# THUDM/CogView

Hardware: AMD Instinct MI355X
Metric: train tokens/sec/node (seq1089, 4B GPT) at 1/2/4/8 MI355X; % MFMA roofline (higher is better)
Workload: dtype fp16

## Files before the change

cogview_amd/_lib.py:

```python
import ctypes as C
import os

_HERE = os.path.dirname(os.path.abspath(__file__))
LIB_PATH = os.environ.get("COGVIEW_HIP_LIB") or os.path.join(_HERE, "lib", "libcogview_hip.so")

F16, BF16, F32 = 0, 1, 2
EPI_BIAS, EPI_GELU, EPI_DGELU, EPI_DROPOUT, EPI_ABSMAX, EPI_ACCUM, EPI_COLSUM = 1, 2, 4, 8, 16, 32, 64
EPI_GELU_DAUX, EPI_MULAUX = 128, 256

_ERR = {1: "bad argument (shape / alignment / dtype)", 2: "kernel launch failure", 3: "unsupported combination"}


class CogviewHipError(RuntimeError):
    pass


class GemmDesc(C.Structure):
    _fields_ = [
        ("dtype", C.c_int), ("trans_a", C.c_int), ("trans_b", C.c_int),
        ("M", C.c_int), ("N", C.c_int), ("K", C.c_int),
        ("A", C.c_void_p), ("lda", C.c_int),
        ("B", C.c_void_p), ("ldb", C.c_int),
        ("C", C.c_void_p), ("ldc", C.c_int),
        ("out_f32", C.c_int), ("flags", C.c_int),
# ... 89 lines not shown


CONV_4X4_S2, CONV_1X1, CONVT_4X4_S2, CONV_3X3_S1 = 0, 1, 2, 3

_vp, _i, _f, _u64, _i64, _sz = C.c_void_p, C.c_int, C.c_float, C.c_uint64, C.c_int64, C.c_size_t

SIGNATURES = {
    "cogv_version": (_i, []),
    "cogv_arch": (C.c_char_p, []),
    "cogv_gemm": (_i, [C.POINTER(GemmDesc), _vp]),
    "cogv_gemm_workspace_bytes": (_sz, [C.POINTER(GemmDesc)]),
    "cogv_gemm_pick_splitk": (_i, [_i, _i, _i]),
    "cogv_gemm_grouped": (_i, [C.POINTER(GemmDesc), _i, _vp]),
    "cogv_gemm_colsum_rows": (_i, [_i]),
    "cogv_colsum_finalize": (_i, [_i, _vp, _i, _i, _vp, _i, _vp]),
    "cogv_gemm_pick_splitk_tiles": (_i, [_i, _i]),
    "cogv_sandwich_ln_fwd": (_i, [_i, _vp, _vp, _vp, _vp, _vp, _vp, _vp, _vp, _vp, _i, _i, _f, _i, _vp]),
    "cogv_sandwich_ln_bwd": (_i, [_i, _vp, _vp, _vp, _vp, _vp, _vp, _vp, _vp, _vp, _vp, _i, _i, _i, _f, _u64, _u64,
                                  _vp, _sz, _i, _vp]),
    "cogv_sandwich_ln_bwd_marked": (_i, [_i, _vp, _vp, _vp, _vp, _vp, _vp, _vp, _vp, _vp, _vp, _i, _i, _i, _f, _vp, _sz, _i, _vp]),
    "cogv_ln_bwd_workspace_bytes": (_sz, [_i, _i]),
    "cogv_sandwich_ln_bwd_pair": (_i, [_i, _vp, _vp, _vp, _vp, _vp, _vp, _vp, _vp, _vp, _vp, _vp, _vp, _vp, _vp, _vp, _vp, _vp, _i, _i, _i, _f,
                                       _vp, _sz, _vp]),
    "cogv_ln_bwd_pair_workspace_bytes": (_sz, [_i, _i]),
    "cogv_ln_bwd_num_blocks": (_i, [_i]),
    "cogv_ln_bwd_plan": (_i, [_i, _i, _i, _f, _i, _i, C.POINTER(C.c_int)]),
    "cogv_ln_bwd_pair_plan": (_i, [_i, _i, _f, C.POINTER(C.c_int)]),
    "cogv_gemm_reserve_cus": (_i, [_i]),
    "cogv_attention_fwd": (_i, [C.POINTER(AttnDesc), _vp]),
    "cogv_attention_bwd": (_i, [C.POINTER(AttnDesc), _vp]),
    "cogv_gemv_ln": (_i, [C.POINTER(GemmDesc), C.POINTER(LnPrologue), _vp]),
    "cogv_gemv_attn": (_i, [C.POINTER(GemmDesc), _vp, _i, _i, _vp]),
    "cogv_attention_decode": (_i, [C.POINTER(AttnDecodeDesc), _vp]),
    "cogv_attention_decode_workspace_bytes": (_sz, [_i, _i, _i]),
    "cogv_attention_keep_bits_bytes": (_sz, [_i, _i, _i, _i]),
    "cogv_sparse_slot_reduce": (_i, [_i, _vp, _vp, _vp, _vp, _vp, _i64, _i, _i64, _i, _i, _i, _i, _i, _i, _i, _vp]),
    "cogv_embedding_fwd": (_i, [_i, _vp, _vp, _i64, _i64, _vp, _vp, _vp, _i64, _vp, _vp, _i64, _i, _f, _u64, _u64, _i, _vp]),
    "cogv_embedding_bwd": (_i, [_i, _vp, _vp, _vp, _i64, _i64, _vp, _vp, _i64, _vp, _i64, _i, _f, _u64, _u64, _vp, _sz, _i, _vp]),
    "cogv_embedding_bwd_workspace_bytes": (_sz, [_i64, _i64]),
    "cogv_gelu_fwd": (_i, [_i, _vp, _vp, _sz, _vp]),
    "cogv_gelu_bwd": (_i, [_i, _vp, _vp, _vp, _sz, _vp]),
    "cogv_dropout": (_i, [_i, _vp, _vp, _sz, _f, _u64, _u64, _vp, _vp]),
    "cogv_add": (_i, [_i, _vp, _vp, _vp, _sz, _vp, _vp]),
    "cogv_add_stream": (_i, [_i, _vp, _vp, _vp, _sz, _vp, _vp]),
    "cogv_scale": (_i, [_i, _vp, _vp, _sz, _f, _vp]),
    "cogv_absmax": (_i, [_i, _vp, _sz, _vp, _vp]),
# ... 41 lines not shown
```

cogview_amd/csrc/layernorm.hip:

```cpp
#include "common.cuh"
#include "cogview_hip.h"

#include <algorithm>
#include <cstdlib>

namespace {

struct LnFwdArgs {
  const void* x; const void* gamma; const void* beta; const void* res;
  void* y; float* mean; float* rstd;
  const float* absmax_in; float* absmax_out;
  int rows, h; float eps;
};

template <typename T, int NV, int MODE>
__global__ __launch_bounds__(256) void ln_fwd_kernel(const LnFwdArgs p) {
  typedef Row8<T, MODE == 1> XR;
  typedef Row8<T, MODE == 2> YR;
  const int lane = threadIdx.x & 63;
  const int wave_global = blockIdx.x * 4 + (threadIdx.x >> 6);
  const int nwaves = gridDim.x * 4;
  float eps = p.eps;
  if (p.absmax_in) { const float c = *p.absmax_in * 0.125f; eps = p.eps * c * c; }
  const float inv_h = 1.0f / (float)p.h;
// ... 332 lines not shown
#endif
      if (act && row < p.rows) {
        float o[8];
#pragma unroll
        for (int i = 0; i < 8; ++i) o[i] = rstd3[r] * fmaf(-xh3[r][i], n2, gy3[r][i] - n1);
        if (p.marked) {
#pragma unroll
          for (int i = 0; i < 8; ++i) o[i] = marked_dropped(aor[r], i) ? 0.f : o[i] * p.keep_scale;
        }
        (void)TR::st(p.d_ao, (size_t)row * p.h + col, o, 0u);
#pragma unroll
        for (int i = 0; i < 8; ++i) cs[i] += o[i];
      }
    }
  }
  if (act) {
    float* o2 = p.partial2 + (size_t)blockIdx.x * 3 * p.h + col;
    float* o3 = p.partial3 + (size_t)blockIdx.x * 3 * p.h + col;
#pragma unroll
    for (int i = 0; i < 8; ++i) { o2[i] = dg2[i]; o2[p.h + i] = db2[i]; o3[i] = dg3[i]; o3[p.h + i] = db3[i]; o3[2 * p.h + i] = cs[i]; }
  }
}

template <typename T>
__global__ __launch_bounds__(1024) void ln_bwd_reduce_kernel(const float* partial, int nblk, int h, void* dgamma,
                                                            void* dbeta, void* colsum, int accumulate) {
  const int c = blockIdx.x * 64 + (threadIdx.x & 63);
  const int part = threadIdx.x >> 6;
  const int set = blockIdx.y;
  T* out = reinterpret_cast<T*>(set == 0 ? dgamma : set == 1 ? dbeta : colsum);
  __shared__ float red[16][64];
  float s = 0.f;
  if (c < h && out) {
    float t[8] = {0.f, 0.f, 0.f, 0.f, 0.f, 0.f, 0.f, 0.f};
    int b = part;
    for (; b + 7 * 16 < nblk; b += 8 * 16) {
#pragma unroll
      for (int u = 0; u < 8; ++u) t[u] += partial[((size_t)(b + 16 * u) * 3 + set) * h + c];
    }
    for (; b < nblk; b += 16) t[0] += partial[((size_t)b * 3 + set) * h + c];
    s = ((t[0] + t[1]) + (t[2] + t[3])) + ((t[4] + t[5]) + (t[6] + t[7]));
  }
  red[part][threadIdx.x & 63] = s;
  __syncthreads();
  if (part == 0 && c < h && out) {
    float t = 0.f;
#pragma unroll
    for (int i = 0; i < 16; ++i) t += red[i][threadIdx.x];
    if (accumulate) t += HT<T>::to_f(out[c]);
    out[c] = HT<T>::from_f(t);
  }
}

template <typename T, int NV, int MODE> void launch_fwd_m(const LnFwdArgs& a, int blocks, hipStream_t st) {
  static const int resident = [] {
    int per_cu = 0, dev = 0;
    hipDeviceProp_t prop;
    if (hipOccupancyMaxActiveBlocksPerMultiprocessor(&per_cu, ln_fwd_kernel<T, NV, MODE>, 256, 0) != hipSuccess || per_cu < 1) return 4096;
    if (hipGetDevice(&dev) != hipSuccess || hipGetDeviceProperties(&prop, dev) != hipSuccess) return 4096;
    return per_cu * prop.multiProcessorCount;
  }();
  if (blocks > resident) blocks = resident;
  hipLaunchKernelGGL((ln_fwd_kernel<T, NV, MODE>), dim3(blocks), dim3(256), 0, st, a);
}
template <typename T, int NV> void launch_fwd(const LnFwdArgs& a, int mode, int blocks, hipStream_t st) {
  if (mode == COGV_LN_STREAM_IN) launch_fwd_m<T, NV, 1>(a, blocks, st);
  else if (mode == COGV_LN_STREAM_OUT) launch_fwd_m<T, NV, 2>(a, blocks, st);
  else launch_fwd_m<T, NV, 0>(a, blocks, st);
}

#define NV_SWITCH(FN, T, nv, ...)                          \
  switch (nv) {                                            \
// ... 33 lines not shown
  if (marked && drop && mode != COGV_LN_STREAM_IN) {
    p.marked = true;
    if (wide && sw.marked_rows != 4) { p.rows_in_flight = 2; p.lean = lean_ok; }
  } else if (lean_ok) { p.rows_in_flight = 2; p.lean = true; }
  else if (wide && (drop || (mode == COGV_LN_STREAM_IN && sw.stream_in_rows == 2))) p.rows_in_flight = 2;
  const int cap = wide ? (p.rows_in_flight == 2 && drop ? 512 : 256) : 2560 / nw;
  p.blocks = p.lean ? ln_bwd_grid(rows, 2, 768) : ln_bwd_grid(rows, 4, cap);
  return p;
}
LnBwdPlan ln_bwd_pair_plan(int rows, int h, bool drop) {
  return LnBwdPlan{2, false, drop, ln_bwd_grid(rows, 2, ln_switches().pair_blocks), 64 * ((h + 511) / 512)};
}

inline bool ln_bwd_args_ok(int mode, int rows, int h, float dropout_p) {
  return mode >= 0 && mode <= 2 && rows > 0 && h > 0 && !(h & 7) && h <= 4096 && dropout_p >= 0.f && dropout_p < 1.f;
}
int ln_plan_out(const LnBwdPlan& p, int out[5]) {
  out[0] = p.rows_in_flight, out[1] = p.lean, out[2] = p.marked, out[3] = p.blocks, out[4] = p.threads;
  return COGV_OK;
}
template <typename T> void ln_bwd_reduce(const float* partial, int nblk, int h, void* dgamma, void* dbeta, void* colsum,
                                         int accumulate, hipStream_t st) {
  if (!dgamma && !dbeta && !colsum) return;
  hipLaunchKernelGGL((ln_bwd_reduce_kernel<T>), dim3((h + 63) / 64, 3), dim3(1024), 0, st, partial, nblk, h, dgamma, dbeta, colsum, accumulate);
}
constexpr int ln_form(int mode, int r, bool lean, bool mark) { return mode * 100 + r * 10 + lean * 2 + mark; }
template <typename T> int ln_bwd_run(const LnBwdArgs& a, int mode, const LnBwdPlan& p, void* dgamma, void* dbeta, void* colsum,
                                     int accumulate, hipStream_t st) {
  switch (ln_form(mode, p.rows_in_flight, p.lean, p.marked)) {
#define LN_FORM(MODE, R, LEAN, MARK) \
  case ln_form(MODE, R, LEAN, MARK): hipLaunchKernelGGL((ln_bwd_kernel<T, R, MODE, LEAN, MARK>), dim3(p.blocks), dim3(p.threads), 0, st, a); break;
    LN_FORM(0, 4, false, false) LN_FORM(0, 2, false, false) LN_FORM(0, 4, false, true) LN_FORM(0, 2, false, true)
    LN_FORM(1, 4, false, false) LN_FORM(1, 2, false, false)
    LN_FORM(2, 4, false, false) LN_FORM(2, 2, false, false) LN_FORM(2, 4, false, true) LN_FORM(2, 2, false, true)
    LN_FORM(2, 2, true, false) LN_FORM(2, 2, true, true)
#undef LN_FORM
    default: return COGV_ERR_UNSUPPORTED;
  }
  ln_bwd_reduce<T>(a.partial, p.blocks, a.h, dgamma, dbeta, colsum, accumulate, st);
  return cogv_check_launch();
}
template <typename T> int ln_bwd_pair_run(const LnPairArgs& a, const LnBwdPlan& p, void* dgamma2, void* dbeta2, void* dgamma3,
                                          void* dbeta3, void* colsum, int accumulate, hipStream_t st) {
  hipLaunchKernelGGL((ln_bwd_pair_kernel<T, 2>), dim3(p.blocks), dim3(p.threads), 0, st, a);
  ln_bwd_reduce<T>(a.partial2, p.blocks, a.h, dgamma2, dbeta2, nullptr, accumulate, st);
  ln_bwd_reduce<T>(a.partial3, p.blocks, a.h, dgamma3, dbeta3, colsum, accumulate, st);
  return cogv_check_launch();
}

}

extern "C" int cogv_ln_bwd_num_blocks(int rows) {
  const int b = (rows + 3) / 4;
  return b < 1 ? 1 : (b > 1024 ? 1024 : b);
}
extern "C" size_t cogv_ln_bwd_workspace_bytes(int rows, int h) {
  return (size_t)cogv_ln_bwd_num_blocks(rows) * 3 * (size_t)h * sizeof(float);
}
extern "C" int cogv_ln_bwd_plan(int stream_mode, int rows, int h, float dropout_p, int marked, int has_add_in, int out[5]) {
  if (marked && stream_mode == COGV_LN_STREAM_IN) return COGV_ERR_ARG;
  if (!ln_bwd_args_ok(stream_mode, rows, h, dropout_p)) return COGV_ERR_ARG;
  return ln_plan_out(ln_bwd_plan(stream_mode, rows, h, ln_thr16(dropout_p) != 0, marked != 0, has_add_in != 0), out);
}
extern "C" int cogv_ln_bwd_pair_plan(int rows, int h, float dropout_p, int out[5]) {
  if (!ln_bwd_args_ok(COGV_LN_ALL_T, rows, h, dropout_p)) return COGV_ERR_ARG;
  if ((h + 511) / 512 < 4) return COGV_ERR_UNSUPPORTED;
  return ln_plan_out(ln_bwd_pair_plan(rows, h, ln_thr16(dropout_p) != 0), out);
}

// ... 33 lines not shown
  return dtype == COGV_F16 ? ln_bwd_run<f16_t>(a, stream_mode, plan, dgamma, dbeta, colsum, accumulate_param_grads, st)
                           : ln_bwd_run<bf16_t>(a, stream_mode, plan, dgamma, dbeta, colsum, accumulate_param_grads, st);
}

extern "C" int cogv_sandwich_ln_bwd(int dtype, const void* dy, const void* x, const void* gamma, const float* mean,
                                    const float* rstd, const void* add_in, void* dx, void* dgamma, void* dbeta,
                                    void* colsum, int accumulate_param_grads, int rows, int h, float dropout_p,
                                    uint64_t seed, uint64_t stream_id, void* workspace, size_t workspace_bytes,
                                    int stream_mode, void* stream) {
  return ln_bwd_impl(dtype, dy, x, gamma, mean, rstd, add_in, dx, dgamma, dbeta, colsum, accumulate_param_grads, rows, h,
                     dropout_p, seed, stream_id, workspace, workspace_bytes, stream_mode, stream, 0);
}

extern "C" int cogv_sandwich_ln_bwd_marked(int dtype, const void* dy, const void* x, const void* gamma, const float* mean,
                                           const float* rstd, const void* add_in, void* dx, void* dgamma, void* dbeta,
                                           void* colsum, int accumulate_param_grads, int rows, int h, float dropout_p,
                                           void* workspace, size_t workspace_bytes, int stream_mode, void* stream) {
  if (stream_mode == COGV_LN_STREAM_IN) return COGV_ERR_ARG;
  return ln_bwd_impl(dtype, dy, x, gamma, mean, rstd, add_in, dx, dgamma, dbeta, colsum, accumulate_param_grads, rows, h,
                     dropout_p, 0, 0, workspace, workspace_bytes, stream_mode, stream, dropout_p > 0.f ? 1 : 0);
}

extern "C" size_t cogv_ln_bwd_pair_workspace_bytes(int rows, int h) { return 2 * cogv_ln_bwd_workspace_bytes(rows, h); }
extern "C" int cogv_sandwich_ln_bwd_pair(int dtype, const void* dc, const void* y, const void* gamma2, const float* mean2,
                                         const float* rstd2, const void* dout, void* dy, void* dgamma2, void* dbeta2,
                                         const void* ao, const void* gamma3, const float* mean3, const float* rstd3, void* d_ao,
                                         void* dgamma3, void* dbeta3, void* colsum, int accumulate_param_grads, int rows, int h,
                                         float dropout_p, void* workspace, size_t workspace_bytes, void* stream) {
  if (dtype != COGV_F16 && dtype != COGV_BF16) return COGV_ERR_UNSUPPORTED;
  if (!ln_bwd_args_ok(COGV_LN_ALL_T, rows, h, dropout_p)) return COGV_ERR_ARG;
  if (!dc || !y || !gamma2 || !mean2 || !rstd2 || !dout || !dy || !ao || !gamma3 || !mean3 || !rstd3 || !d_ao || !workspace) return COGV_ERR_ARG;
  if (workspace_bytes < cogv_ln_bwd_pair_workspace_bytes(rows, h)) return COGV_ERR_ARG;
  if (((uintptr_t)dc | (uintptr_t)y | (uintptr_t)gamma2 | (uintptr_t)dout | (uintptr_t)dy | (uintptr_t)ao | (uintptr_t)gamma3 | (uintptr_t)d_ao) & 15)
    return COGV_ERR_ARG;
  if ((h + 511) / 512 < 4) return COGV_ERR_UNSUPPORTED;
  const uint32_t thr16 = ln_thr16(dropout_p);
  float* const partial = reinterpret_cast<float*>(workspace);
  const LnPairArgs a{dc, y, gamma2, mean2, rstd2, dout, dy, ao, gamma3, mean3, rstd3, d_ao, partial,
                     partial + (size_t)cogv_ln_bwd_num_blocks(rows) * 3 * (size_t)h, rows, h, thr16 != 0, 65536.0f / (65536.0f - (float)thr16)};
  const LnBwdPlan plan = ln_bwd_pair_plan(rows, h, thr16 != 0);
  hipStream_t st = reinterpret_cast<hipStream_t>(stream);
  return dtype == COGV_F16 ? ln_bwd_pair_run<f16_t>(a, plan, dgamma2, dbeta2, dgamma3, dbeta3, colsum, accumulate_param_grads, st)
                           : ln_bwd_pair_run<bf16_t>(a, plan, dgamma2, dbeta2, dgamma3, dbeta3, colsum, accumulate_param_grads, st);
}
```

cogview_amd/functional.py:

```python
import contextlib
import math
import os

import torch

from . import ops
from .mpu import mappings
from .mpu import random as mpu_random
from .mpu.initialize import get_model_parallel_group, mp_rank_or_0, mp_world_size_or_1


def grad_buffer(p):
    if p.grad is None:
        p.grad = torch.zeros_like(p)
    return p.grad


def grad_accumulate(*params):
    params = [p for p in params if p is not None]
    arenas = [getattr(p, "_cogv_arena", (None,))[0] for p in params]
    if params and all(a is not None and a is arenas[0] for a in arenas):
        return not arenas[0].take_fresh(params)
    for p, a in zip(params, arenas):
        if a is not None:
            a.ensure_zeroed(p)
# ... 487 lines not shown
                                    slot_ao, residual=x, absmax_out=slot_y, save_stats=keep is not None)
    c, m2, r2 = ops.sandwich_ln_fwd(y, layer.post_attention_layernorm.weight, layer.post_attention_layernorm.bias,
                                    eps, slot_y, save_stats=keep is not None)
    f4 = mlp_m.dense_h_to_4h.weight.shape[0]
    u = torch.empty((rows, f4), dtype=a.dtype, device=dev) if keep is not None else None
    g = ops.gemm(c.view(rows, h), mlp_m.dense_h_to_4h.weight, bias=mlp_m.dense_h_to_4h.bias, gelu=True, gelu_daux=u)
    slot_mo = ops.new_absmax_slot(dev)
    if mp == 1:
        mo = ops.gemm(g, mlp_m.dense_4h_to_h.weight, bias=mlp_m.dense_4h_to_h.bias, dropout=d_mo, absmax=slot_mo)
    else:
        mo = _row_parallel_chunked(g, mlp_m.dense_4h_to_h.weight, mlp_m.dense_4h_to_h.bias if rank == 0 else None, d_mo, slot_mo)
    slot_out = ops.new_absmax_slot(dev)
    out, m4, r4 = ops.sandwich_ln_fwd(mo.view(b, s, h), layer.fourth_layernorm.weight, layer.fourth_layernorm.bias,
                                      eps, slot_mo, residual=y, absmax_out=slot_out, save_stats=keep is not None)
    if keep is not None:
        keep.x, keep.a, keep.qkv, keep.att, keep.lse, keep.ao, keep.y, keep.c = x, a, qkv, att, lse, ao, y, c
        keep.u, keep.g, keep.mo = u, g, mo
        keep.st1, keep.st2, keep.st3, keep.st4 = (m1, r1), (m2, r2), (m3, r3), (m4, r4)
        keep.d_attn, keep.d_ao, keep.d_mo, keep.kbits = d_attn, d_ao, d_mo, kbits
    return out, slot_out


LN_BWD_PAIR = os.environ.get("COGV_LN_BWD_PAIR", "1") != "0"


def _layer_backward(layer, kp, dout, sep):
    att_m, mlp_m = layer.attention, layer.mlp
    b, s, h = kp.x.shape
    rows = b * s
    npp = att_m.num_attention_heads_per_partition
    hp = npp * 64
    G = grad_buffer
    ln1, ln2, ln3, ln4 = (layer.input_layernorm, layer.post_attention_layernorm, layer.third_layernorm,
                          layer.fourth_layernorm)
    W1, b1, W2, b2 = mlp_m.dense_h_to_4h.weight, mlp_m.dense_h_to_4h.bias, mlp_m.dense_4h_to_h.weight, mlp_m.dense_4h_to_h.bias
    Wq, bq, Wo, bo = att_m.query_key_value.weight, att_m.query_key_value.bias, att_m.dense.weight, att_m.dense.bias
    dout = dout if dout.is_contiguous() else dout.contiguous()

    marked = mp_world_size_or_1() == 1 and os.environ.get("COGV_LN_BWD_MARKED", "1") != "0"
    d_mo = ops.sandwich_ln_bwd(dout, kp.mo, ln4.weight, *kp.st4, dropout=kp.d_mo, dgamma=G(ln4.weight), marked=marked,
                               dbeta=G(ln4.bias), colsum=G(b2), accumulate=grad_accumulate(ln4.weight, ln4.bias, b2)).view(rows, h)
    mp = mp_world_size_or_1()
    wgrads = []

    def _wg(dy_, x_, w_):
        if mp == 1:
            defer_weight_grad(dy_, x_, w_, owner=layer)
        else:
            wgrads.append((dy_, x_, w_))
    du = ops.gemm(d_mo, W2, trans_b=True, mul_aux=kp.u, colsum_out=G(b1),
                  colsum_accumulate=grad_accumulate(b1))
    _wg(d_mo, kp.g, W2)
    dc = ops.gemm(du, W1, trans_b=True)
    _wg(du, kp.c.view(rows, h), W1)
    if mp > 1:
        work = _mp_allreduce_start(dc)
        with _room_for_collective():
            _launch_weight_grads(wgrads)
        del wgrads[:]
        _mp_allreduce_finish(work)
    p_ao = 0.0 if kp.d_ao is None else float(kp.d_ao[0])
    if LN_BWD_PAIR and ops.ln_bwd_pair_supported(h) and (marked or p_ao == 0.0):
        dy, d_ao = ops.sandwich_ln_bwd_pair(dc.view(b, s, h), kp.y, ln2.weight, *kp.st2, dout, kp.ao, ln3.weight, *kp.st3,
                                            dropout_p=p_ao, dgamma2=G(ln2.weight), dbeta2=G(ln2.bias), dgamma3=G(ln3.weight),
# ... 4 lines not shown
        dy = ops.sandwich_ln_bwd(dc.view(b, s, h), kp.y, ln2.weight, *kp.st2, add_in=dout, dgamma=G(ln2.weight),
                                 dbeta=G(ln2.bias), accumulate=grad_accumulate(ln2.weight, ln2.bias))
        d_ao = ops.sandwich_ln_bwd(dy, kp.ao, ln3.weight, *kp.st3, dropout=kp.d_ao, dgamma=G(ln3.weight), marked=marked,
                                   dbeta=G(ln3.bias), colsum=G(bo), accumulate=grad_accumulate(ln3.weight, ln3.bias, bo)).view(rows, h)
    d_att = ops.gemm(d_ao, Wo, trans_b=True).view(b, s, npp, 64)
    _wg(d_ao, kp.att.view(rows, hp), Wo)
    qkv = kp.qkv
    q = qkv[:, :, 0:hp].view(b, s, npp, 64)
    k = qkv[:, :, hp:2 * hp].view(b, s, npp, 64)
    v = qkv[:, :, 2 * hp:].view(b, s, npp, 64)
    dqkv = torch.empty_like(qkv)
    ops.attention_bwd(d_att, q, k, v, kp.att, kp.lse, sep=sep, dropout=kp.d_attn,
                      dq=dqkv[:, :, 0:hp].view(b, s, npp, 64), dk=dqkv[:, :, hp:2 * hp].view(b, s, npp, 64),
                      dv=dqkv[:, :, 2 * hp:].view(b, s, npp, 64), colsum_out=G(bq), colsum_accumulate=grad_accumulate(bq),
                      keep_bits=getattr(kp, "kbits", None))
    dqkv2 = dqkv.view(rows, 3 * hp)
    da = ops.gemm(dqkv2, Wq, trans_b=True)
    _wg(dqkv2, kp.a.view(rows, h), Wq)
    if mp > 1:
        work = _mp_allreduce_start(da)
        with _room_for_collective():
            _launch_weight_grads(wgrads)
        _mp_allreduce_finish(work)
    dx = ops.sandwich_ln_bwd(da.view(b, s, h), kp.x, ln1.weight, *kp.st1, add_in=dy, dgamma=G(ln1.weight),
                             dbeta=G(ln1.bias), accumulate=grad_accumulate(ln1.weight, ln1.bias))
    return dx


class _WgradEntry:
    __slots__ = ("dy", "x", "w", "owner", "t0", "trows", "tiles_n", "acc")

    def __init__(self, dy, x, w, owner):
        self.dy, self.x, self.w, self.owner = dy, x, w, owner
        self.t0, self.acc = 0, None
        self.trows, self.tiles_n = (w.shape[0] + 255) // 256, (w.shape[1] + 255) // 256

    def tiles_left(self):
        return (self.trows - self.t0) * self.tiles_n


def plan_wgrad_chunks(entries, budget):
    out, left = [], budget
    for i, (t0, trows, tiles_n, out_rows) in enumerate(entries):
        if t0 >= trows:
            continue
        n = trows - t0
# ... 106 lines not shown
def nested_backward():
    _NESTED_OUTER.append(torch._C._current_graph_task_id())
    try:
        yield
    finally:
        _NESTED_OUTER.pop()


def defer_weight_grad(dy, x, w, owner=None):
    q = _WGRADS
    task = torch._C._current_graph_task_id()
    root = _NESTED_OUTER[0] if _NESTED_OUTER else task
    if root >= 0 and q.root != root:
        q.entries, q.callbacks, q.new_tiles = [], [], 0
        q.root, q.hooked = root, set()
    if task >= 0 and task not in q.hooked:
        torch.autograd.Variable._execution_engine.queue_callback(_flush_at_end_of_backward)
        q.hooked.add(task)
    q.add(dy, x, w, owner)


class _TransformerLayer(torch.autograd.Function):
    @staticmethod
    def forward(ctx, x, absmax_x, layer, sep, drops, recompute, on_backward_done):
        xc = x if x.is_contiguous() else x.contiguous()
        keep = None if recompute else _LayerCtx()
        out, slot = _layer_forward(layer, xc, absmax_x, sep, drops, keep)
        ctx.layer, ctx.sep, ctx.drops, ctx.recompute, ctx.keep = layer, sep, drops, recompute, keep
        ctx.done_cb = on_backward_done
        if recompute:
            piece, ctx.x_shape = mpu_random.partition_activation(xc)
            ctx.save_for_backward(piece, absmax_x)
        ctx.mark_non_differentiable(slot)
        return out, slot

    @staticmethod
    def backward(ctx, dout, _):
        keep = ctx.keep
        if ctx.recompute:
            xc, absmax_x = ctx.saved_tensors
            xc = mpu_random.gather_activation(xc, ctx.x_shape)
            keep = _LayerCtx()
            _layer_forward(ctx.layer, xc, absmax_x, ctx.sep, ctx.drops, keep)
        dx = _layer_backward(ctx.layer, keep, dout, ctx.sep)
        ctx.keep = None
        if ctx.done_cb is not None:
            _WGRADS.callbacks.append((ctx.done_cb, ctx.layer))
        idx = getattr(ctx.layer, "_cogv_index", 0)
        if idx % wgrad_group_layers(ctx.layer) == 0:
            flush_weight_grads(final=(idx == 0))
        return dx, None, None, None, None, None, None


_DECODE_FUSE_ENV = _os.environ.get("COGV_DECODE_FUSE_COMBINE")


_DECODE_CHAIN_MAX_ROWS = min(8, max(0, int(_os.environ.get("COGV_DECODE_CHAIN_MAX_ROWS", "4"))))


def _decode_fuse_combine():
    if _DECODE_FUSE_ENV is not None:
        return _DECODE_FUSE_ENV != "0"
    return not torch.cuda.is_current_stream_capturing()


def decode_chain_supported(tr, batch):
    h = tr.layers[0].input_layernorm.weight.shape[0]
    return (mp_world_size_or_1() == 1 and batch <= _DECODE_CHAIN_MAX_ROWS and h % 512 == 0 and h <= 4096
            and tr.layers[0].input_layernorm.weight.dtype in (torch.float16, torch.bfloat16))


def decode_chain(tr, h0, absmax0, slots, emb_weight):
    b, s, h = h0.shape
    assert s == 1
# ... 22 lines not shown
        z, z_absmax, post, res = mo, None, (layer.fourth_layernorm.weight, layer.fourth_layernorm.bias), y
    fl = tr.final_layernorm
    logits, _ = ops.gemv_ln(z, emb_weight, None, fl.weight, fl.bias, fl.eps, z_absmax, post, res)
    return logits.view(b, 1, emb_weight.shape[0])


def transformer_layer_kv(layer, x, absmax_x, sep, kv_slot):
    xc = x if x.is_contiguous() else x.contiguous()
    if absmax_x is None:
        absmax_x = ops.absmax(xc)
    out, slot = _layer_forward(layer, xc, absmax_x, sep, (None, None, None), None, kv_slot=kv_slot)
    out._cogv_absmax = slot
    return out


def transformer_layer(layer, x, absmax_x, sep, training, recompute=False, on_backward_done=None):
    p_attn = layer.attention.attention_dropout.p
    p_out = layer.attention.output_dropout.p
    p_mlp = layer.mlp.dropout.p
    drops = (_drop(p_attn, training, attention=True), _drop(p_out, training), _drop(p_mlp, training))
    if absmax_x is None:
        absmax_x = ops.absmax(x if x.is_contiguous() else x.contiguous())
    if torch.is_grad_enabled() and x.requires_grad:
        out, slot = _TransformerLayer.apply(x, absmax_x, layer, sep, drops, recompute, on_backward_done)
    else:
        out, slot = _layer_forward(layer, x if x.is_contiguous() else x.contiguous(), absmax_x, sep, drops, None)
    out._cogv_absmax = slot
    return out
```

cogview_amd/ops.py:

```python
import ctypes as C
import os

import torch

from . import _lib as L

_DT = {torch.float16: L.F16, torch.bfloat16: L.BF16, torch.float32: L.F32}


def dt_code(t):
    try:
        return _DT[t.dtype if isinstance(t, torch.Tensor) else t]
    except KeyError:
        raise L.CogviewHipError(f"unsupported dtype {t.dtype if isinstance(t, torch.Tensor) else t}")


def _need_gpu(*ts):
    for t in ts:
        if t is not None and not t.is_cuda:
            raise L.CogviewHipError(
                "cogview_amd ops run only on an MI355X (HIP) device: got a CPU tensor and there is no CPU fallback")


def _p(t):
# ... 420 lines not shown

def sandwich_ln_bwd_pair(dc, y, gamma2, mean2, rstd2, dout, ao, gamma3, mean3, rstd3, dropout_p=0.0, dgamma2=None, dbeta2=None,
                         dgamma3=None, dbeta3=None, colsum=None, accumulate=False):
    _need_gpu(dc, y, ao)
    h = y.shape[-1]
    dc2, y2, do2, ao2 = dc.reshape(-1, h), y.reshape(-1, h), dout.reshape(-1, h), ao.reshape(-1, h)
    assert dc2.is_contiguous() and y2.is_contiguous() and do2.is_contiguous() and ao2.is_contiguous()
    if y.dtype != torch.float32 or dout.dtype != torch.float32 or dc.dtype != gamma2.dtype or ao.dtype != gamma2.dtype:
        raise L.CogviewHipError("Sandwich-LN backward pair: y / dout must be the fp32 stream, dc / ao the 16-bit storage type")
    rows = y2.shape[0]
    dy = torch.empty_like(y2)
    d_ao = torch.empty_like(ao2)
    lib = L.lib()
    ws = workspace("ln_bwd_pair", lib.cogv_ln_bwd_pair_workspace_bytes(rows, h), y.device)
    nb = rows * h * (2 + 4 + 4 + 4 + 2 + 2)
    with timed_launch("layernorm", 0.0, nb, lambda: "ln_bwd pair: stream in + add, then stream out" + (" + dropout from marked zeros" if dropout_p > 0.0 else "")):
        L.check(lib.cogv_sandwich_ln_bwd_pair(dt_code(gamma2), _p(dc2), _p(y2), _p(gamma2), _p(mean2), _p(rstd2), _p(do2), _p(dy),
                                              _p(dgamma2), _p(dbeta2), _p(ao2), _p(gamma3), _p(mean3), _p(rstd3), _p(d_ao),
                                              _p(dgamma3), _p(dbeta3), _p(colsum), int(accumulate), rows, h, float(dropout_p),
                                              _p(ws), ws.numel(), _stream()), "cogv_sandwich_ln_bwd_pair")
    return dy.view(y.shape), d_ao.view(ao.shape)


def attention_executed_flops(b, H, s_q, s_k, sep=0, dense=True):
    nq, nk = (s_q + 63) // 64, (s_k + 63) // 64
    if dense:
        off = s_k - s_q
        sep_i = int(sep) if isinstance(sep, int) else 0
        blocks = 0
        for i in range(nq):
            last_key = max(min(s_q, 64 * i + 64) - 1 + off, sep_i - 1)
            blocks += max(0, min(nk, last_key // 64 + 1))
    else:
        blocks = nq * nk
    return float(b) * H * blocks * 4.0 * 64 * 64 * 64


def _attn_strides(t):
    assert t.dim() == 4 and t.shape[-1] == 64 and t.stride(3) == 1 and (t.stride(2) == 64 or t.shape[2] == 1)
    return t.stride(0), t.stride(1)


def _attn_desc(q, k, v, o, sep, dropout):
    d = L.AttnDesc()
    d.dtype = dt_code(q)
    d.B, d.s_q, d.H = q.shape[0], q.shape[1], q.shape[2]
# ... 436 lines not shown
```

include/cogview_hip.h:

```cpp
#ifndef COGVIEW_HIP_H
#define COGVIEW_HIP_H

#include <stddef.h>
#include <stdint.h>

#ifdef __cplusplus
extern "C" {
#endif

#define COGV_F16 0
#define COGV_BF16 1
#define COGV_F32 2

int cogv_version(void);
const char* cogv_arch(void);

#define COGV_EPI_BIAS 1
#define COGV_EPI_GELU 2
#define COGV_EPI_DGELU 4
#define COGV_EPI_DROPOUT 8
#define COGV_EPI_ABSMAX 16
#define COGV_EPI_ACCUM 32
#define COGV_EPI_COLSUM 64

// ... 38 lines not shown
} cogv_ln_prologue;
int cogv_gemv_ln(const cogv_gemm_desc* d, const cogv_ln_prologue* ln, void* stream);
int cogv_gemv_attn(const cogv_gemm_desc* d, const void* partials, int heads, int capacity, void* stream);

#define COGV_LN_ALL_T 0
#define COGV_LN_STREAM_IN 1
#define COGV_LN_STREAM_OUT 2
int cogv_sandwich_ln_fwd(int dtype, const void* x, const void* gamma, const void* beta, const void* residual,
                         void* y, float* mean, float* rstd, const float* absmax_in, float* absmax_out,
                         int rows, int h, float eps, int stream_mode, void* stream);
int cogv_sandwich_ln_bwd(int dtype, const void* dy, const void* x, const void* gamma, const float* mean,
                         const float* rstd, const void* add_in, void* dx, void* dgamma, void* dbeta, void* colsum,
                         int accumulate_param_grads, int rows, int h, float dropout_p, uint64_t seed,
                         uint64_t stream_id, void* workspace, size_t workspace_bytes, int stream_mode, void* stream);
int cogv_sandwich_ln_bwd_marked(int dtype, const void* dy, const void* x, const void* gamma, const float* mean,
                                const float* rstd, const void* add_in, void* dx, void* dgamma, void* dbeta, void* colsum,
                                int accumulate_param_grads, int rows, int h, float dropout_p, void* workspace,
                                size_t workspace_bytes, int stream_mode, void* stream);
int cogv_sandwich_ln_bwd_pair(int dtype, const void* dc, const void* y, const void* gamma2, const float* mean2,
                              const float* rstd2, const void* dout, void* dy, void* dgamma2, void* dbeta2,
                              const void* ao, const void* gamma3, const float* mean3, const float* rstd3, void* d_ao,
                              void* dgamma3, void* dbeta3, void* colsum, int accumulate_param_grads, int rows, int h,
                              float dropout_p, void* workspace, size_t workspace_bytes, void* stream);
size_t cogv_ln_bwd_pair_workspace_bytes(int rows, int h);
size_t cogv_ln_bwd_workspace_bytes(int rows, int h);
int cogv_ln_bwd_num_blocks(int rows);
int cogv_ln_bwd_plan(int stream_mode, int rows, int h, float dropout_p, int marked, int has_add_in, int out[5]);
int cogv_ln_bwd_pair_plan(int rows, int h, float dropout_p, int out[5]);

typedef struct cogv_attn_desc {
  int dtype; int B, H, s_q, s_k, head_dim; int sep;
  float scale;
  float dropout_p; uint64_t seed; uint64_t stream_id;
  const void* q; const void* k; const void* v; void* o;
  const void* dout; void* dq; void* dk; void* dv;
  float* lse; float* dvec;
  long long q_bs, k_bs, v_bs, o_bs, do_bs, dq_bs, dk_bs, dv_bs;
  int q_rs, k_rs, v_rs, o_rs, do_rs, dq_rs, dk_rs, dv_rs;
  float* colsum_partial;
  const int* kv_index; long long kv_index_bs;
  long long kv_index_gs; int sparse_window, sparse_pivots; float sparse_pivot_bias;
  void* keep_bits;
  const void* mask; long long mask_bs;
} cogv_attn_desc;
int cogv_attention_fwd(const cogv_attn_desc* d, void* stream);
int cogv_attention_bwd(const cogv_attn_desc* d, void* stream);
// ... 104 lines not shown
```

Measured before the change: 43980.

## Pair LN1 backward with the layer below's LN4 backward across layer boundaries

Fuses the current layer's LN1 backward with the next-lower layer's LN4 backward into one pair kernel. It hands the resulting d_mo and the un-reduced partial sums down to that layer, which then runs only the parameter-grad reduction instead of a full LN4 backward pass. The non-open pair path also merges its two reduce launches into a single 6-set reduce kernel. The aim is to cut a memory-bound LN pass and launches per layer, at the cost of cross-layer state, an extra partial buffer allocation per layer, and a fallback path when the gradient identity check fails.

```diff
diff --git a/cogview_amd/_lib.py b/cogview_amd/_lib.py
--- a/cogview_amd/_lib.py
+++ b/cogview_amd/_lib.py
@@ -135,6 +135,9 @@
     "cogv_ln_bwd_workspace_bytes": (_sz, [_i, _i]),
     "cogv_sandwich_ln_bwd_pair": (_i, [_i, _vp, _vp, _vp, _vp, _vp, _vp, _vp, _vp, _vp, _vp, _vp, _vp, _vp, _vp, _vp, _vp, _vp, _i, _i, _i, _f,
                                        _vp, _sz, _vp]),
+    "cogv_sandwich_ln_bwd_pair_open": (_i, [_i, _vp, _vp, _vp, _vp, _vp, _vp, _vp, _vp, _vp, _i, _vp, _vp, _vp, _vp, _vp, _vp, _sz, _i, _i, _f,
+                                            _vp, _sz, _vp]),
+    "cogv_ln_bwd_reduce": (_i, [_i, _vp, _i, _i, _vp, _vp, _vp, _i, _vp]),
     "cogv_ln_bwd_pair_workspace_bytes": (_sz, [_i, _i]),
     "cogv_ln_bwd_num_blocks": (_i, [_i]),
     "cogv_ln_bwd_plan": (_i, [_i, _i, _i, _f, _i, _i, C.POINTER(C.c_int)]),
diff --git a/cogview_amd/csrc/layernorm.hip b/cogview_amd/csrc/layernorm.hip
--- a/cogview_amd/csrc/layernorm.hip
+++ b/cogview_amd/csrc/layernorm.hip
@@ -378,16 +378,23 @@
   }
 }
 
+struct LnReduceArgs {
+  const float* partial[2];
+  void* out[6];
+  int nblk, h, accumulate[2];
+};
 template <typename T>
-__global__ __launch_bounds__(1024) void ln_bwd_reduce_kernel(const float* partial, int nblk, int h, void* dgamma,
-                                                            void* dbeta, void* colsum, int accumulate) {
+__global__ __launch_bounds__(1024) void ln_bwd_reduce_kernel(const LnReduceArgs a) {
   const int c = blockIdx.x * 64 + (threadIdx.x & 63);
   const int part = threadIdx.x >> 6;
-  const int set = blockIdx.y;
-  T* out = reinterpret_cast<T*>(set == 0 ? dgamma : set == 1 ? dbeta : colsum);
+  const int which = blockIdx.y / 3, set = blockIdx.y % 3;
+  const float* partial = a.partial[which];
+  const int nblk = a.nblk, h = a.h;
+  T* out = reinterpret_cast<T*>(a.out[blockIdx.y]);
+  if (!out) return;
   __shared__ float red[16][64];
   float s = 0.f;
-  if (c < h && out) {
+  if (c < h) {
     float t[8] = {0.f, 0.f, 0.f, 0.f, 0.f, 0.f, 0.f, 0.f};
     int b = part;
     for (; b + 7 * 16 < nblk; b += 8 * 16) {
@@ -399,11 +406,11 @@
   }
   red[part][threadIdx.x & 63] = s;
   __syncthreads();
-  if (part == 0 && c < h && out) {
+  if (part == 0 && c < h) {
     float t = 0.f;
 #pragma unroll
     for (int i = 0; i < 16; ++i) t += red[i][threadIdx.x];
-    if (accumulate) t += HT<T>::to_f(out[c]);
+    if (a.accumulate[which]) t += HT<T>::to_f(out[c]);
     out[c] = HT<T>::from_f(t);
   }
 }
@@ -483,7 +490,8 @@
 template <typename T> void ln_bwd_reduce(const float* partial, int nblk, int h, void* dgamma, void* dbeta, void* colsum,
                                          int accumulate, hipStream_t st) {
   if (!dgamma && !dbeta && !colsum) return;
-  hipLaunchKernelGGL((ln_bwd_reduce_kernel<T>), dim3((h + 63) / 64, 3), dim3(1024), 0, st, partial, nblk, h, dgamma, dbeta, colsum, accumulate);
+  const LnReduceArgs a{{partial, nullptr}, {dgamma, dbeta, colsum, nullptr, nullptr, nullptr}, nblk, h, {accumulate, 0}};
+  hipLaunchKernelGGL((ln_bwd_reduce_kernel<T>), dim3((h + 63) / 64, 3), dim3(1024), 0, st, a);
 }
 constexpr int ln_form(int mode, int r, bool lean, bool mark) { return mode * 100 + r * 10 + lean * 2 + mark; }
 template <typename T> int ln_bwd_run(const LnBwdArgs& a, int mode, const LnBwdPlan& p, void* dgamma, void* dbeta, void* colsum,
@@ -502,10 +510,13 @@
   return cogv_check_launch();
 }
 template <typename T> int ln_bwd_pair_run(const LnPairArgs& a, const LnBwdPlan& p, void* dgamma2, void* dbeta2, void* dgamma3,
-                                          void* dbeta3, void* colsum, int accumulate, hipStream_t st) {
+                                          void* dbeta3, void* colsum, int accumulate, bool open, hipStream_t st) {
   hipLaunchKernelGGL((ln_bwd_pair_kernel<T, 2>), dim3(p.blocks), dim3(p.threads), 0, st, a);
-  ln_bwd_reduce<T>(a.partial2, p.blocks, a.h, dgamma2, dbeta2, nullptr, accumulate, st);
-  ln_bwd_reduce<T>(a.partial3, p.blocks, a.h, dgamma3, dbeta3, colsum, accumulate, st);
+  if (open) ln_bwd_reduce<T>(a.partial2, p.blocks, a.h, dgamma2, dbeta2, nullptr, accumulate, st);
+  else if (dgamma2 || dbeta2 || dgamma3 || dbeta3 || colsum) {
+    const LnReduceArgs r{{a.partial2, a.partial3}, {dgamma2, dbeta2, nullptr, dgamma3, dbeta3, colsum}, p.blocks, a.h, {accumulate, accumulate}};
+    hipLaunchKernelGGL((ln_bwd_reduce_kernel<T>), dim3((a.h + 63) / 64, 6), dim3(1024), 0, st, r);
+  }
   return cogv_check_launch();
 }
 
@@ -585,24 +596,53 @@
 }
 
 extern "C" size_t cogv_ln_bwd_pair_workspace_bytes(int rows, int h) { return 2 * cogv_ln_bwd_workspace_bytes(rows, h); }
+static int ln_bwd_pair_impl(int dtype, const void* dc, const void* y, const void* gamma2, const float* mean2,
+                            const float* rstd2, const void* dout, void* dy, void* dgamma2, void* dbeta2,
+                            const void* ao, const void* gamma3, const float* mean3, const float* rstd3, void* d_ao,
+                            void* dgamma3, void* dbeta3, void* colsum, int accumulate_param_grads, int rows, int h,
+                            float dropout_p, float* partial3, void* workspace, size_t workspace_bytes, void* stream) {
+  if (dtype != COGV_F16 && dtype != COGV_BF16) return COGV_ERR_UNSUPPORTED;
+  if (!ln_bwd_args_ok(COGV_LN_ALL_T, rows, h, dropout_p)) return COGV_ERR_ARG;
+  if (!dc || !y || !gamma2 || !mean2 || !rstd2 || !dout || !dy || !ao || !gamma3 || !mean3 || !rstd3 || !d_ao || !workspace) return COGV_ERR_ARG;
+  if (workspace_bytes < (partial3 ? cogv_ln_bwd_workspace_bytes(rows, h) : cogv_ln_bwd_pair_workspace_bytes(rows, h))) return COGV_ERR_ARG;
+  if (((uintptr_t)dc | (uintptr_t)y | (uintptr_t)gamma2 | (uintptr_t)dout | (uintptr_t)dy | (uintptr_t)ao | (uintptr_t)gamma3 | (uintptr_t)d_ao |
+       (uintptr_t)partial3) & 15)
+    return COGV_ERR_ARG;
+  if ((h + 511) / 512 < 4) return COGV_ERR_UNSUPPORTED;
+  const uint32_t thr16 = ln_thr16(dropout_p);
+  float* const partial = reinterpret_cast<float*>(workspace);
+  const bool open = partial3 != nullptr;
+  const LnPairArgs a{dc, y, gamma2, mean2, rstd2, dout, dy, ao, gamma3, mean3, rstd3, d_ao, partial,
+                     open ? partial3 : partial + (size_t)cogv_ln_bwd_num_blocks(rows) * 3 * (size_t)h, rows, h, thr16 != 0,
+                     65536.0f / (65536.0f - (float)thr16)};
+  const LnBwdPlan plan = ln_bwd_pair_plan(rows, h, thr16 != 0);
+  hipStream_t st = reinterpret_cast<hipStream_t>(stream);
+  return dtype == COGV_F16 ? ln_bwd_pair_run<f16_t>(a, plan, dgamma2, dbeta2, dgamma3, dbeta3, colsum, accumulate_param_grads, open, st)
+                           : ln_bwd_pair_run<bf16_t>(a, plan, dgamma2, dbeta2, dgamma3, dbeta3, colsum, accumulate_param_grads, open, st);
+}
 extern "C" int cogv_sandwich_ln_bwd_pair(int dtype, const void* dc, const void* y, const void* gamma2, const float* mean2,
                                          const float* rstd2, const void* dout, void* dy, void* dgamma2, void* dbeta2,
                                          const void* ao, const void* gamma3, const float* mean3, const float* rstd3, void* d_ao,
                                          void* dgamma3, void* dbeta3, void* colsum, int accumulate_param_grads, int rows, int h,
                                          float dropout_p, void* workspace, size_t workspace_bytes, void* stream) {
+  return ln_bwd_pair_impl(dtype, dc, y, gamma2, mean2, rstd2, dout, dy, dgamma2, dbeta2, ao, gamma3, mean3, rstd3, d_ao, dgamma3,
+                          dbeta3, colsum, accumulate_param_grads, rows, h, dropout_p, nullptr, workspace, workspace_bytes, stream);
+}
+extern "C" int cogv_sandwich_ln_bwd_pair_open(int dtype, const void* da, const void* x, const void* gamma1, const float* mean1,
+                                              const float* rstd1, const void* add_in, void* dx, void* dgamma1, void* dbeta1,
+                                              int accumulate_param_grads, const void* mo, const void* gamma4, const float* mean4,
+                                              const float* rstd4, void* d_mo, float* partial4, size_t partial4_bytes, int rows,
+                                              int h, float dropout_p, void* workspace, size_t workspace_bytes, void* stream) {
+  if (!partial4 || partial4_bytes < cogv_ln_bwd_workspace_bytes(rows, h)) return COGV_ERR_ARG;
+  return ln_bwd_pair_impl(dtype, da, x, gamma1, mean1, rstd1, add_in, dx, dgamma1, dbeta1, mo, gamma4, mean4, rstd4, d_mo, nullptr,
+                          nullptr, nullptr, accumulate_param_grads, rows, h, dropout_p, partial4, workspace, workspace_bytes, stream);
+}
+extern "C" int cogv_ln_bwd_reduce(int dtype, const float* partial, int nblk, int h, void* dgamma, void* dbeta, void* colsum,
+                                  int accumulate_param_grads, void* stream) {
   if (dtype != COGV_F16 && dtype != COGV_BF16) return COGV_ERR_UNSUPPORTED;
-  if (!ln_bwd_args_ok(COGV_LN_ALL_T, rows, h, dropout_p)) return COGV_ERR_ARG;
-  if (!dc || !y || !gamma2 || !mean2 || !rstd2 || !dout || !dy || !ao || !gamma3 || !mean3 || !rstd3 || !d_ao || !workspace) return COGV_ERR_ARG;
-  if (workspace_bytes < cogv_ln_bwd_pair_workspace_bytes(rows, h)) return COGV_ERR_ARG;
-  if (((uintptr_t)dc | (uintptr_t)y | (uintptr_t)gamma2 | (uintptr_t)dout | (uintptr_t)dy | (uintptr_t)ao | (uintptr_t)gamma3 | (uintptr_t)d_ao) & 15)
-    return COGV_ERR_ARG;
-  if ((h + 511) / 512 < 4) return COGV_ERR_UNSUPPORTED;
-  const uint32_t thr16 = ln_thr16(dropout_p);
-  float* const partial = reinterpret_cast<float*>(workspace);
-  const LnPairArgs a{dc, y, gamma2, mean2, rstd2, dout, dy, ao, gamma3, mean3, rstd3, d_ao, partial,
-                     partial + (size_t)cogv_ln_bwd_num_blocks(rows) * 3 * (size_t)h, rows, h, thr16 != 0, 65536.0f / (65536.0f - (float)thr16)};
-  const LnBwdPlan plan = ln_bwd_pair_plan(rows, h, thr16 != 0);
+  if (!partial || nblk <= 0 || nblk > 1024 || h <= 0 || (h & 7) || h > 4096) return COGV_ERR_ARG;
   hipStream_t st = reinterpret_cast<hipStream_t>(stream);
-  return dtype == COGV_F16 ? ln_bwd_pair_run<f16_t>(a, plan, dgamma2, dbeta2, dgamma3, dbeta3, colsum, accumulate_param_grads, st)
-                           : ln_bwd_pair_run<bf16_t>(a, plan, dgamma2, dbeta2, dgamma3, dbeta3, colsum, accumulate_param_grads, st);
-}
+  if (dtype == COGV_F16) ln_bwd_reduce<f16_t>(partial, nblk, h, dgamma, dbeta, colsum, accumulate_param_grads, st);
+  else ln_bwd_reduce<bf16_t>(partial, nblk, h, dgamma, dbeta, colsum, accumulate_param_grads, st);
+  return cogv_check_launch();
+}
diff --git a/cogview_amd/functional.py b/cogview_amd/functional.py
--- a/cogview_amd/functional.py
+++ b/cogview_amd/functional.py
@@ -1,6 +1,7 @@
 import contextlib
 import math
 import os
+import warnings
 
 import torch
 
@@ -534,9 +535,32 @@
 
 
 LN_BWD_PAIR = os.environ.get("COGV_LN_BWD_PAIR", "1") != "0"
-
-
-def _layer_backward(layer, kp, dout, sep):
+LN_BWD_BOUNDARY_PAIR = os.environ.get("COGV_LN_BWD_BOUNDARY_PAIR", "1") != "0"
+BOUNDARY_PAIR_STATS = {"paired": 0, "claimed": 0, "unclaimed": 0}
+
+
+class _Boundary:
+    __slots__ = ("layer", "keep", "ahead")
+
+    def __init__(self, layer):
+        self.layer, self.keep, self.ahead = layer, None, None
+
+    def claim(self, dout):
+        ahead, self.ahead = self.ahead, None
+        if ahead is None:
+            return None
+        dx, version, d_mo, pending = ahead
+        if (dout.data_ptr() == dx.data_ptr() and dout.shape == dx.shape and dout.dtype == dx.dtype and dout.stride() == dx.stride()
+                and dout._version == version == dx._version):
+            BOUNDARY_PAIR_STATS["claimed"] += 1
+            return d_mo, pending
+        BOUNDARY_PAIR_STATS["unclaimed"] += 1
+        warnings.warn("Sandwich-LN boundary pair: the gradient a layer received is not the one the layer above handed down; "
+                      "its LN4 backward runs on its own (COGV_LN_BWD_BOUNDARY_PAIR=0 avoids the lost work)")
+        return None
+
+
+def _layer_backward(layer, kp, dout, sep, below=None, link=None):
     att_m, mlp_m = layer.attention, layer.mlp
     b, s, h = kp.x.shape
     rows = b * s
@@ -550,8 +574,15 @@
     dout = dout if dout.is_contiguous() else dout.contiguous()
 
     marked = mp_world_size_or_1() == 1 and os.environ.get("COGV_LN_BWD_MARKED", "1") != "0"
-    d_mo = ops.sandwich_ln_bwd(dout, kp.mo, ln4.weight, *kp.st4, dropout=kp.d_mo, dgamma=G(ln4.weight), marked=marked,
-                               dbeta=G(ln4.bias), colsum=G(b2), accumulate=grad_accumulate(ln4.weight, ln4.bias, b2)).view(rows, h)
+    ahead = link.claim(dout) if link is not None else None
+    if ahead is not None:
+        d_mo, pending = ahead
+        ops.ln_bwd_reduce(pending, dgamma=G(ln4.weight), dbeta=G(ln4.bias), colsum=G(b2), accumulate=grad_accumulate(ln4.weight, ln4.bias, b2))
+        d_mo = d_mo.view(rows, h)
+        del ahead, pending
+    else:
+        d_mo = ops.sandwich_ln_bwd(dout, kp.mo, ln4.weight, *kp.st4, dropout=kp.d_mo, dgamma=G(ln4.weight), marked=marked,
+                                   dbeta=G(ln4.bias), colsum=G(b2), accumulate=grad_accumulate(ln4.weight, ln4.bias, b2)).view(rows, h)
     mp = mp_world_size_or_1()
     wgrads = []
 
@@ -602,6 +633,18 @@
         with _room_for_collective():
             _launch_weight_grads(wgrads)
         _mp_allreduce_finish(work)
+    lo = below.keep if below is not None else None
+    if (LN_BWD_BOUNDARY_PAIR and lo is not None and mp == 1 and ops.ln_bwd_boundary_pair_supported(h, kp.x)
+            and lo.mo.shape[-1] == h and lo.mo.numel() == kp.x.numel()):
+        p_mo = 0.0 if lo.d_mo is None else float(lo.d_mo[0])
+        if marked or p_mo == 0.0:
+            lo_ln4 = below.layer.fourth_layernorm
+            dx, d_mo_lo, pending = ops.sandwich_ln_bwd_pair_open(da.view(b, s, h), kp.x, ln1.weight, *kp.st1, dy, lo.mo, lo_ln4.weight,
+                                                                 *lo.st4, dropout_p=p_mo, dgamma1=G(ln1.weight), dbeta1=G(ln1.bias),
+                                                                 accumulate=grad_accumulate(ln1.weight, ln1.bias))
+            below.ahead = (dx, dx._version, d_mo_lo, pending)
+            BOUNDARY_PAIR_STATS["paired"] += 1
+            return dx
     dx = ops.sandwich_ln_bwd(da.view(b, s, h), kp.x, ln1.weight, *kp.st1, add_in=dy, dgamma=G(ln1.weight),
                              dbeta=G(ln1.bias), accumulate=grad_accumulate(ln1.weight, ln1.bias))
     return dx
@@ -754,11 +797,14 @@
 
 class _TransformerLayer(torch.autograd.Function):
     @staticmethod
-    def forward(ctx, x, absmax_x, layer, sep, drops, recompute, on_backward_done):
+    def forward(ctx, x, absmax_x, layer, sep, drops, recompute, on_backward_done, below=None, link=None):
         xc = x if x.is_contiguous() else x.contiguous()
         keep = None if recompute else _LayerCtx()
         out, slot = _layer_forward(layer, xc, absmax_x, sep, drops, keep)
         ctx.layer, ctx.sep, ctx.drops, ctx.recompute, ctx.keep = layer, sep, drops, recompute, keep
+        ctx.below, ctx.link = (below if xc is x and not recompute else None), link
+        if link is not None:
+            link.keep = keep
         ctx.done_cb = on_backward_done
         if recompute:
             piece, ctx.x_shape = mpu_random.partition_activation(xc)
@@ -774,14 +820,17 @@
             xc = mpu_random.gather_activation(xc, ctx.x_shape)
             keep = _LayerCtx()
             _layer_forward(ctx.layer, xc, absmax_x, ctx.sep, ctx.drops, keep)
-        dx = _layer_backward(ctx.layer, keep, dout, ctx.sep)
+        dx = _layer_backward(ctx.layer, keep, dout, ctx.sep, ctx.below, ctx.link)
         ctx.keep = None
+        if ctx.link is not None:
+            ctx.link.keep = None
+        ctx.below = ctx.link = None
         if ctx.done_cb is not None:
             _WGRADS.callbacks.append((ctx.done_cb, ctx.layer))
         idx = getattr(ctx.layer, "_cogv_index", 0)
         if idx % wgrad_group_layers(ctx.layer) == 0:
             flush_weight_grads(final=(idx == 0))
-        return dx, None, None, None, None, None, None
+        return dx, None, None, None, None, None, None, None, None
 
 
 _DECODE_FUSE_ENV = _os.environ.get("COGV_DECODE_FUSE_COMBINE")
@@ -850,7 +899,10 @@
     if absmax_x is None:
         absmax_x = ops.absmax(x if x.is_contiguous() else x.contiguous())
     if torch.is_grad_enabled() and x.requires_grad:
-        out, slot = _TransformerLayer.apply(x, absmax_x, layer, sep, drops, recompute, on_backward_done)
+        below = getattr(x, "_cogv_boundary", None) if LN_BWD_BOUNDARY_PAIR else None
+        link = _Boundary(layer) if LN_BWD_BOUNDARY_PAIR else None
+        out, slot = _TransformerLayer.apply(x, absmax_x, layer, sep, drops, recompute, on_backward_done, below, link)
+        out._cogv_boundary = link
     else:
         out, slot = _layer_forward(layer, x if x.is_contiguous() else x.contiguous(), absmax_x, sep, drops, None)
     out._cogv_absmax = slot
diff --git a/cogview_amd/ops.py b/cogview_amd/ops.py
--- a/cogview_amd/ops.py
+++ b/cogview_amd/ops.py
@@ -466,6 +466,46 @@
     return dy.view(y.shape), d_ao.view(ao.shape)
 
 
+def ln_bwd_boundary_pair_supported(h, t):
+    return ln_bwd_pair_supported(h) and t.is_cuda
+
+
+def sandwich_ln_bwd_pair_open(da, x, gamma1, mean1, rstd1, add_in, mo, gamma4, mean4, rstd4, dropout_p=0.0, dgamma1=None,
+                              dbeta1=None, accumulate=False):
+    _need_gpu(da, x, mo)
+    h = x.shape[-1]
+    da2, x2, ad2, mo2 = da.reshape(-1, h), x.reshape(-1, h), add_in.reshape(-1, h), mo.reshape(-1, h)
+    assert da2.is_contiguous() and x2.is_contiguous() and ad2.is_contiguous() and mo2.is_contiguous()
+    if x.dtype != torch.float32 or add_in.dtype != torch.float32 or da.dtype != gamma1.dtype or mo.dtype != gamma1.dtype:
+        raise L.CogviewHipError("Sandwich-LN backward pair: x / add_in must be the fp32 stream, da / mo the 16-bit storage type")
+    rows = x2.shape[0]
+    dx = torch.empty_like(x2)
+    d_mo = torch.empty_like(mo2)
+    lib = L.lib()
+    plan = (C.c_int * 5)()
+    L.check(lib.cogv_ln_bwd_pair_plan(rows, h, float(dropout_p), plan), "cogv_ln_bwd_pair_plan")
+    partial = torch.empty(lib.cogv_ln_bwd_workspace_bytes(rows, h) // 4, dtype=torch.float32, device=x.device)
+    ws = workspace("ln_bwd", lib.cogv_ln_bwd_workspace_bytes(rows, h), x.device)
+    nb = rows * h * (2 + 4 + 4 + 4 + 2 + 2)
+    with timed_launch("layernorm", 0.0, nb, lambda: "ln_bwd boundary pair: stream in + add, then stream out" + (" + dropout from marked zeros" if dropout_p > 0.0 else "")):
+        L.check(lib.cogv_sandwich_ln_bwd_pair_open(dt_code(gamma1), _p(da2), _p(x2), _p(gamma1), _p(mean1), _p(rstd1), _p(ad2), _p(dx),
+                                                   _p(dgamma1), _p(dbeta1), int(accumulate), _p(mo2), _p(gamma4), _p(mean4), _p(rstd4),
+                                                   _p(d_mo), _p(partial), partial.numel() * 4, rows, h, float(dropout_p),
+                                                   _p(ws), ws.numel(), _stream()), "cogv_sandwich_ln_bwd_pair_open")
+    return dx.view(x.shape), d_mo.view(mo.shape), (partial, int(plan[3]), h, gamma4.dtype)
+
+
+def ln_bwd_reduce(pending, dgamma=None, dbeta=None, colsum=None, accumulate=False):
+    partial, nblk, h, dtype = pending
+    outs = [t for t in (dgamma, dbeta, colsum) if t is not None]
+    if not outs:
+        return
+    if any(t.dtype != dtype or t.numel() != h for t in outs):
+        raise L.CogviewHipError("Sandwich-LN backward reduce: outputs must be [h] tensors of the storage type")
+    L.check(L.lib().cogv_ln_bwd_reduce(dt_code(outs[0]), _p(partial), nblk, h, _p(dgamma), _p(dbeta), _p(colsum), int(accumulate),
+                                       _stream()), "cogv_ln_bwd_reduce")
+
+
 def attention_executed_flops(b, H, s_q, s_k, sep=0, dense=True):
     nq, nk = (s_q + 63) // 64, (s_k + 63) // 64
     if dense:
diff --git a/include/cogview_hip.h b/include/cogview_hip.h
--- a/include/cogview_hip.h
+++ b/include/cogview_hip.h
@@ -84,6 +84,13 @@
                               const void* ao, const void* gamma3, const float* mean3, const float* rstd3, void* d_ao,
                               void* dgamma3, void* dbeta3, void* colsum, int accumulate_param_grads, int rows, int h,
                               float dropout_p, void* workspace, size_t workspace_bytes, void* stream);
+int cogv_sandwich_ln_bwd_pair_open(int dtype, const void* da, const void* x, const void* gamma1, const float* mean1,
+                                   const float* rstd1, const void* add_in, void* dx, void* dgamma1, void* dbeta1,
+                                   int accumulate_param_grads, const void* mo, const void* gamma4, const float* mean4,
+                                   const float* rstd4, void* d_mo, float* partial4, size_t partial4_bytes, int rows, int h,
+                                   float dropout_p, void* workspace, size_t workspace_bytes, void* stream);
+int cogv_ln_bwd_reduce(int dtype, const float* partial, int nblk, int h, void* dgamma, void* dbeta, void* colsum,
+                       int accumulate_param_grads, void* stream);
 size_t cogv_ln_bwd_pair_workspace_bytes(int rows, int h);
 size_t cogv_ln_bwd_workspace_bytes(int rows, int h);
 int cogv_ln_bwd_num_blocks(int rows);
```

Result: no change. 44230, median of 6 (+0.6%).
